# kornelski/cavif-rs

Hardware: AMD Instinct MI355X
Metric: MPix/s encoded at speed=4 q=80, 1080p batch; bit-exact vs CPU oracle (higher is better)
Workload: dtype u16 samples / i32 transform / i64 RD cost

## Files before the change

### __graft_entry__.py

```python
import os
import subprocess
import sys

ROOT = os.path.dirname(os.path.abspath(__file__))
sys.path.insert(0, ROOT)

HIPCC_FLAGS = ['--offload-arch=gfx950', '-O2', '-mllvm', '-sink-insts-to-avoid-spills', '-mllvm', '-inline-threshold=1000', '-mllvm', '-disable-machine-licm', '-mllvm', '-phi-node-folding-threshold=1', '-std=c++17', '-ffp-contract=off', '-fPIC', '-shared', '-Wno-unused-variable']


def _digest(sources, flags):
    import hashlib
    h = hashlib.sha256(' '.join(flags).encode())
    for s in sorted(sources):
        with open(s, 'rb') as fh:
            h.update(os.path.basename(s).encode() + b'\0' + fh.read())
    return h.hexdigest()


def _stale(target, sources):
    if not os.path.exists(target):
        return True
    t = os.path.getmtime(target)
    return any(os.path.getmtime(s) > t for s in sources)

# ... 9 lines not shown
        subprocess.check_call([hipcc] + HIPCC_FLAGS + ['-o', out, os.path.join(csrc, 'mi_avif.hip'), '-lz'])
        with open(stamp, 'w') as fh:
            fh.write(want + '\n')
    cli_src = os.path.join(ROOT, 'cavif_rs_amd', 'cli', 'cavif_mi.cpp')
    cli = os.path.join(ROOT, 'cavif_rs_amd', 'cavif_mi')
    if force or _stale(cli, [cli_src, out, os.path.join(ROOT, 'include', 'mi_avif.h')]):
        subprocess.check_call(['g++', '-O2', '-std=c++17', '-o', cli, cli_src, '-L' + os.path.join(ROOT, 'cavif_rs_amd'), '-lmi_avif', '-lpthread', '-Wl,-rpath,$ORIGIN'])
    subprocess.check_call(['make', '-s', '-C', os.path.join(ROOT, 'oracle')])
    try:
        from tests import emu
        emu.build(force=force)
    except Exception as e:
        print('warning: tests/emu build failed (%s); the -m "not gpu" emulator tests will fail, the product library is unaffected' % e, file=sys.stderr)
    try:
        from tests.helpers import k4_harness
        k4_harness.build_all(force=force)
    except Exception as e:
        print('warning: tests/kernels harness build failed (%s); tests/test_k4_coder.py will fail, the product library is unaffected' % e, file=sys.stderr)
    try:
        from tests.helpers import filters_harness
        filters_harness.build_all(force=force)
    except Exception as e:
        print('warning: tests/kernels filter harness build failed (%s); tests/test_loopfilter_kernels.py will fail, the product library is unaffected' % e, file=sys.stderr)
    try:
        from tests.helpers import predict_harness
        predict_harness.build_all(force=force)
    except Exception as e:
        print('warning: tests/kernels prediction harness build failed (%s); tests/test_predict_kernels.py will fail, the product library is unaffected' % e, file=sys.stderr)
    try:
        from tests.helpers import k1_lookups_harness
        k1_lookups_harness.build_all(force=force)
    except Exception as e:
        print('warning: tests/kernels lookup harness build failed (%s); tests/test_k1_lookups.py will fail, the product library is unaffected' % e, file=sys.stderr)
    import cavif_rs_amd
    cavif_rs_amd.load_library()


def smoke():
    import numpy as np
    import cavif_rs_amd as m
    from cavif_rs_amd.synth import synth_image
    from tests.helpers import oracle
    assert m.device_count() >= 1, 'no HIP device visible'
    img = synth_image(256, 192, index=3)
    enc = m.Encoder().with_quality(80).with_speed(4).with_bit_depth(10)
    got = enc.encode_rgb(img)
    ref, cs, _ = oracle.ravif_encode(img, quality=80, speed=4, depth=10)
    assert got.avif_file[4:12] == b'ftypavif'
    assert got.avif_file == ref, 'HIP path and CPU oracle disagree (%d vs %d bytes)' % (len(got.avif_file), len(ref))
    print('smoke ok: %dx%d -> %d bytes (colour %d), identical to the oracle' % (img.shape[1], img.shape[0], len(got.avif_file), got.color_byte_size))


if __name__ == '__main__':
    build(force='--force' in sys.argv)
    if '--smoke' in sys.argv:
        smoke()
```

### cavif_rs_amd/csrc/dev_common.h

```cpp
#pragma once
#include <hip/hip_runtime.h>
#include <stdint.h>
#include <stddef.h>
#include "av1_tables.h"

#define MI_TX_DEPTH_MAX 2
#define MI_MAX_TILE_COLS 64
#define MI_MAX_TILE_ROWS 64

enum { BS_4 = 0, BS_8 = 1, BS_16 = 2, BS_32 = 3, BS_64 = 4 };
enum { BS_4X8 = 5, BS_8X4 = 6 };
enum { DC_PRED = 0, V_PRED, H_PRED, D45_PRED, D135_PRED, D113_PRED, D157_PRED, D203_PRED, D67_PRED,
       SMOOTH_PRED, SMOOTH_V_PRED, SMOOTH_H_PRED, PAETH_PRED, UV_CFL_PRED };
enum { DCT_DCT = 0, ADST_DCT, DCT_ADST, ADST_ADST, FLIPADST_DCT, DCT_FLIPADST, FLIPADST_FLIPADST,
       ADST_FLIPADST, FLIPADST_ADST, IDTX, V_DCT, H_DCT, V_ADST, H_ADST, V_FLIPADST, H_FLIPADST };
enum { TXC_2D = 0, TXC_HORIZ = 1, TXC_VERT = 2 };

#define MI_SEG_BINS 4096
struct SegTab {
  int n, mean, thr[7], qidx[8], pad_[3];
  struct Q { int dc_q[3], ac_q[3]; uint32_t dc_recip[3], ac_recip[3]; } q[8];
};
struct FrameDev {
  int w, h, bd, np;
// ... 56 lines not shown
__device__ __forceinline__ int imax_(int a, int b) { return a > b ? a : b; }
__device__ __forceinline__ int iclamp_(int v, int lo, int hi) { return v < lo ? lo : (v > hi ? hi : v); }
__device__ __forceinline__ int iabs_(int a) { return a < 0 ? -a : a; }
__device__ __forceinline__ int round2_(int x, int n) { return n == 0 ? x : (x + (1 << (n - 1))) >> n; }
__device__ __forceinline__ int dim_wl(int code) { return code <= 4 ? 2 + code : (code == 5 ? 2 : 3); }
__device__ __forceinline__ int dim_hl(int code) { return code <= 4 ? 2 + code : (code == 5 ? 3 : 2); }

__device__ __forceinline__ int lut4(unsigned long long tab, int i) { return (int)((tab >> (4 * i)) & 15); }
__device__ __forceinline__ int lut8(unsigned long long tab, int i) { return (int)((tab >> (8 * i)) & 255); }
__device__ __forceinline__ int mode_angle_of(int m) { return m == 8 ? 67 : lut8(0xcb9d71872db45a00ULL, m); }
__device__ __forceinline__ int intra_mode_ctx(int m) { return lut4(0x210344443210ULL, m); }

__device__ __forceinline__ int uni32(int v) { return __builtin_amdgcn_readfirstlane(v); }
__device__ __forceinline__ long long uni64(long long v) {
  return (long long)(((unsigned long long)(uint32_t)uni32((int)((unsigned long long)v >> 32)) << 32) | (uint32_t)uni32((int)v));
}

#define DPP_(old, v, ctrl, rmask) __builtin_amdgcn_update_dpp((int)(old), (int)(v), (ctrl), (rmask), 0xF, false)
__device__ __forceinline__ int wave_sum_i32(int v) {
  v += DPP_(0, v, 0xB1, 0xF); v += DPP_(0, v, 0x4E, 0xF); v += DPP_(0, v, 0x141, 0xF); v += DPP_(0, v, 0x140, 0xF);
  v += DPP_(0, v, 0x142, 0xA); v += DPP_(0, v, 0x143, 0xC);
  return __builtin_amdgcn_readlane(v, 63);
}
__device__ __forceinline__ int wave_max_i32(int v) {
  v = imax_(v, DPP_(v, v, 0xB1, 0xF)); v = imax_(v, DPP_(v, v, 0x4E, 0xF)); v = imax_(v, DPP_(v, v, 0x141, 0xF)); v = imax_(v, DPP_(v, v, 0x140, 0xF));
  v = imax_(v, DPP_(v, v, 0x142, 0xA)); v = imax_(v, DPP_(v, v, 0x143, 0xC));
  return __builtin_amdgcn_readlane(v, 63);
}
__device__ __forceinline__ int wave_or_i32(int v) {
  v |= DPP_(0, v, 0xB1, 0xF); v |= DPP_(0, v, 0x4E, 0xF); v |= DPP_(0, v, 0x141, 0xF); v |= DPP_(0, v, 0x140, 0xF);
  v |= DPP_(0, v, 0x142, 0xA); v |= DPP_(0, v, 0x143, 0xC);
  return __builtin_amdgcn_readlane(v, 63);
}
__device__ __forceinline__ long long wave_sum_i64(long long v) {
  const int lo = wave_sum_i32((int)(v & 0xFFFFFF)), hi = wave_sum_i32((int)(v >> 24));
  return ((long long)hi << 24) + (long long)lo;
}
#define WAVE_SYNC() do { __builtin_amdgcn_fence(__ATOMIC_ACQ_REL, "wavefront"); __builtin_amdgcn_wave_barrier(); } while (0)
#define WG_SYNC() __syncthreads()

struct TileB { int mi_row_start, mi_row_end, mi_col_start, mi_col_end; };

__device__ __forceinline__ int seg_ilog2_q11(uint32_t x) {
  if (x == 0) x = 1;
  const int msb = 31 - __clz((int)x);
  unsigned long long m = (unsigned long long)x << (31 - msb);
  int frac = 0;
#pragma unroll
  for (int i = 0; i < 11; i++) { m = (m * m) >> 31; frac <<= 1; if (m >> 32) { frac |= 1; m >>= 1; } }
  return (msb << 11) | frac;
}
__device__ __forceinline__ int seg_bucket(uint32_t scale_q14) { return iclamp_((seg_ilog2_q11(scale_q14) - (6 << 11)) >> 3, 0, MI_SEG_BINS - 1); }
__device__ __forceinline__ int seg_pred(int ul, int u, int l, int *ctx) {
  *ctx = ul < 0 ? 0 : ((ul == u && ul == l) ? 2 : ((ul == u || ul == l || u == l) ? 1 : 0));
  if (u == -1) return l == -1 ? 0 : l;
  if (l == -1) return u;
  return ul == u ? u : l;
}
__device__ __forceinline__ int seg_neg_deinterleave(int diff, int ref, int max) {
  if (!ref) return diff;
  if (ref >= max - 1) return max - diff - 1;
  if (2 * ref < max) { if (diff <= 2 * ref) return (diff & 1) ? ref + ((diff + 1) >> 1) : ref - (diff >> 1); return diff; }
  if (diff <= 2 * (max - ref - 1)) return (diff & 1) ? ref + ((diff + 1) >> 1) : ref - (diff >> 1);
  return max - (diff + 1);
}
__device__ __forceinline__ int seg_symbol(int seg, int pred, int max) {
// ... 91 lines not shown
```

### cavif_rs_amd/csrc/dev_group.h

```cpp
#pragma once
#include "dev_predict.h"
#include "dev_txfm.h"
#include "dev_rate.h"

struct GroupBuf8 {
  int32_t tbuf[8 * 9];
  int32_t cbuf[64];
  int32_t qc[64];
  uint16_t rec[64];
  uint8_t lev[144];
};
#define GROUP_LANE (LANE & 15)
#define GROUP_ID (LANE >> 4)

template <int CTRL> __device__ __forceinline__ int dpp_row_(int v) { return __builtin_amdgcn_update_dpp(0, v, CTRL, 0xF, 0xF, false); }
__device__ __forceinline__ int row_sum_i32(int v) { v += dpp_row_<0x128>(v); v += dpp_row_<0x124>(v); v += dpp_row_<0x122>(v); v += dpp_row_<0x121>(v); return v; }
__device__ __forceinline__ int row_max_i32(int v) {
  v = imax_(v, dpp_row_<0x128>(v)); v = imax_(v, dpp_row_<0x124>(v)); v = imax_(v, dpp_row_<0x122>(v)); v = imax_(v, dpp_row_<0x121>(v)); return v;
}

static __device__ const int tx4_tab[2][3][4][8] = {
  { { { 2896, 2896, 2896, 2896, 0, 0, 0, 0 }, { 3784, 1567, -1567, -3784, 0, 0, 0, 0 }, { 2896, -2896, -2896, 2896, 0, 0, 0, 0 }, { 1567, -3784, 3784, -1567, 0, 0, 0, 0 } },
    { { 1321, 2482, 3344, 3803, 0, 0, 0, 0 }, { 3344, 3344, 0, -3344, 0, 0, 0, 0 }, { 3803, -1321, -3344, 2482, 0, 0, 0, 0 }, { 2482, -3803, 3344, -1321, 0, 0, 0, 0 } },
    { { 5793, 0, 0, 0, 0, 0, 0, 0 }, { 0, 5793, 0, 0, 0, 0, 0, 0 }, { 0, 0, 5793, 0, 0, 0, 0, 0 }, { 0, 0, 0, 5793, 0, 0, 0, 0 } } },
// ... 329 lines not shown
    buf[i - 1] = (uint16_t)((s + 8) >> 4);
  }
  WAVE_SYNC();
}
__device__ __forceinline__ void edge_upsample_group(LDS uint16_t *buf, int num_px, int on, int bd, LDS uint16_t *tmp, int gl) {
  if (on) for (int i = gl; i < num_px + 3; i += 16) {
    uint16_t v;
    if (i == 0) v = buf[-1]; else if (i == num_px + 2) v = buf[num_px - 1]; else v = buf[i - 2];
    tmp[i] = v;
  }
  WAVE_SYNC();
  const int mx = (1 << bd) - 1;
  if (on) {
    if (gl == 0) buf[-2] = tmp[0];
    for (int i = gl; i < num_px; i += 16) {
      int s = -(int)tmp[i] + 9 * (int)tmp[i + 1] + 9 * (int)tmp[i + 2] - (int)tmp[i + 3];
      s = iclamp_(round2_(s, 4), 0, mx);
      buf[2 * i - 1] = (uint16_t)s;
      buf[2 * i] = tmp[i + 2];
    }
  }
  WAVE_SYNC();
}

template <int N>
__device__ inline void predict_dir_group(const LDS FrameDev *f, int x, int y, int have_left, int have_above, int pa, int ftype,
                                         const LDS uint16_t *ra, const LDS uint16_t *rl, LDS GroupPredBuf *gp, LDS uint16_t *out = nullptr) {
  constexpr int log2w = N == 4 ? 2 : 3, nn = N * N;
  const int gl = GROUP_LANE, bd = f->bd;
  const int max_x = f->mi_cols * 4 - 1, max_y = f->mi_rows * 4 - 1;
  LDS uint16_t *wa = gp->wa + EDGE_OFF, *wl = gp->wl + EDGE_OFF;
  for (int i = gl; i < 2 * N + 1; i += 16) { wa[i - 1] = ra[i - 1]; wl[i - 1] = rl[i - 1]; }
  WAVE_SYNC();
  const int diag = pa != 90 && pa != 180;
  {
    const int st_a = (diag && have_above) ? edge_strength_dev(N, N, ftype, pa - 90) : 0;
    const int num_a = imin_(N, max_x - x + 1) + (pa < 90 ? N : 0) + 1;
    edge_filter_group(wa, num_a, st_a, gp->tmp, gl);
    const int st_l = (diag && have_left) ? edge_strength_dev(N, N, ftype, pa - 180) : 0;
    const int num_l = imin_(N, max_y - y + 1) + (pa > 180 ? N : 0) + 1;
    edge_filter_group(wl, num_l, st_l, gp->tmp, gl);
  }
  const int up_a = edge_upsample_sel_dev(N, N, ftype, pa - 90);
  edge_upsample_group(wa, N + (pa < 90 ? N : 0), up_a, bd, gp->tmp, gl);
  const int up_l = edge_upsample_sel_dev(N, N, ftype, pa - 180);
  edge_upsample_group(wl, N + (pa > 180 ? N : 0), up_l, bd, gp->tmp, gl);
  int dx = 0, dy = 0;
#pragma unroll
  for (int r = 0; r < 4; r++) {
    int sdx, sdy;
    dr_dxdy_uni(__builtin_amdgcn_readlane(pa, 16 * r), &sdx, &sdy);
    dx = GROUP_ID == r ? sdx : dx; dy = GROUP_ID == r ? sdy : dy;
  }
  for (int idx = gl; idx < nn; idx += 16) {
    const int i = idx >> log2w, j = idx & (N - 1);
    int v;
    if (pa < 90) {
      const int max_base = (2 * N - 1) << up_a;
      const int id = (i + 1) * dx, base = (id >> (6 - up_a)) + (j << up_a), sh = ((id << up_a) >> 1) & 0x1F;
      v = base < max_base ? round2_(wa[base] * (32 - sh) + wa[base + 1] * sh, 5) : wa[max_base];
    } else if (pa > 90 && pa < 180) {
      int id = (j << 6) - (i + 1) * dx, base = id >> (6 - up_a);
      if (base >= -(1 << up_a)) { const int sh = ((id << up_a) >> 1) & 0x1F; v = round2_(wa[base] * (32 - sh) + wa[base + 1] * sh, 5); }
      else { id = (i << 6) - (j + 1) * dy; base = id >> (6 - up_l); const int sh = ((id << up_l) >> 1) & 0x1F; v = round2_(wl[base] * (32 - sh) + wl[base + 1] * sh, 5); }
    } else if (pa > 180) {
      const int id = (j + 1) * dy, base = (id >> (6 - up_l)) + (i << up_l), sh = ((id << up_l) >> 1) & 0x1F;
      v = round2_(wl[base] * (32 - sh) + wl[base + 1] * sh, 5);
    } else if (pa == 90) v = wa[j];
    else v = wl[i];
    (out ? out : (LDS uint16_t *)gp->pred)[idx] = (uint16_t)v;
  }
  WAVE_SYNC();
}

template <int N>
__device__ inline void predict_nondir_group(int mode, int have_left, int have_above, int bd, const LDS uint16_t *ra, const LDS uint16_t *rl, LDS uint16_t *pred) {
  constexpr int log2w = N == 4 ? 2 : 3, IT = N * N / 16;
  constexpr unsigned long long wt = N == 4 ? 0x405595FFULL : 0x202532496992C5FFULL;
  const int gl = GROUP_LANE;
  if (mode == DC_PRED) {
    int v = 1 << (bd - 1);
    if (have_left || have_above) {
      int s = gl < N ? (have_above ? (int)ra[gl] : 0) + (have_left ? (int)rl[gl] : 0) : 0;
      s = row_sum_i32(s);
      v = (have_left && have_above) ? (s + N) >> (log2w + 1) : (s + (N >> 1)) >> log2w;
    }
// ... 53 lines not shown
```

### cavif_rs_amd/csrc/dev_predict.h

```cpp
#pragma once
#include "dev_common.h"

#define EDGE_OFF 16
#define EDGE_LEN(N) (EDGE_OFF + 2 * (N) + 16)

__device__ __forceinline__ const uint8_t *sm_weights_dev(int log2w) {
  static __device__ const uint8_t sw[124] = { 255, 149, 85, 64,
                                              255, 197, 146, 105, 73, 50, 37, 32,
                                              255, 225, 196, 170, 145, 123, 102, 84, 68, 54, 43, 33, 26, 20, 17, 16,
                                              255, 240, 225, 210, 196, 182, 169, 157, 145, 133, 122, 111, 101, 92, 83, 74,
                                              66, 59, 52, 45, 39, 34, 29, 25, 21, 17, 14, 12, 10, 9, 8, 8,
                                              255, 248, 240, 233, 225, 218, 210, 203, 196, 189, 182, 176, 169, 163, 156, 150,
                                              144, 138, 133, 127, 121, 116, 111, 106, 101, 96, 91, 86, 82, 77, 73, 69,
                                              65, 61, 57, 54, 50, 47, 44, 41, 38, 35, 32, 29, 27, 25, 22, 20,
                                              18, 16, 15, 13, 12, 10, 9, 8, 7, 6, 6, 5, 5, 4, 4, 4 };
  const int l = ((log2w >= 2) & (log2w <= 5)) ? log2w : 6;
  return sw + ((1 << l) - 4);
}
__device__ __forceinline__ int dr_deriv_dev(int a) {
  const int aa = (unsigned)a < 90u ? a : 0;
  const int k = (aa * 43) >> 7;
  const unsigned long long w01 = k < 8 ? 0x97b2d7117423ff00ULL : 0x4047505a00667484ULL, w23 = k < 24 ? 0x171b1f23282d3339ULL : 0x000003070b000f13ULL;
  const unsigned long long w = k < 16 ? w01 : w23;
  const int v = lut8(w, k & 7) | ((int)((0x16cULL >> (2 * k)) & 3) << 8);
  const int r = (int)((0xf035554000eaaa03ULL >> (2 * k)) & 3);
  return aa - 3 * k == r ? v : 0;
}
__device__ __forceinline__ int edge_strength_dev(int w, int h, int ft, int delta) {
  const int d = imin_(iabs_(delta), 254), blk = w + h;
  const int c = (blk > 8) + (blk > 12) + (blk > 16) + (blk > 24) + (blk > 32);
  const unsigned long long t1 = ft == 0 ? 0x010108282838ULL : 0x010104141428ULL, t2 = ft == 0 ? 0x010410ffffffULL : 0x010104303040ULL;
  const unsigned long long t3 = ft == 0 ? 0x012020ffffffULL : 0x010104ffffffULL;
  return (d >= lut8(t1, c)) + (d >= lut8(t2, c)) + (d >= lut8(t3, c));
}
__device__ __forceinline__ int edge_upsample_sel_dev(int w, int h, int ft, int delta) {
  const int d = iabs_(delta), blk = w + h;
  return (int)((d > 0) & (d < 40) & (blk <= (ft == 0 ? 16 : 8)));
}
__device__ __forceinline__ void dr_dxdy_dev(int pa, int *dx, int *dy) {
  *dx = dr_deriv_dev(pa < 90 ? pa : 180 - pa);
  *dy = dr_deriv_dev(pa < 180 ? pa - 90 : 270 - pa);
}
static __device__ const uint32_t dr_dxdy_tab[91] = {
    0x300000, 0x0003ff, 0x000223, 0x000174, 0x200111, 0x2000d7, 0x2000b2, 0x200097, 0x200084, 0x200074, 0x200066, 0x300000, 0x00005a,
    0x000050, 0x000047, 0x000040, 0x000039, 0x000033, 0x00002d, 0x100028, 0x100023, 0x10001f, 0x10001b, 0x100017, 0x100013, 0x10000f,
    0x300000, 0x00000b, 0x000007, 0x000003, 0x300000, 0x0ffc03, 0x088c07, 0x05d00b, 0x24440f, 0x235c13, 0x22c817, 0x225c1b, 0x22101f,
    0x21d023, 0x219828, 0x300000, 0x01682d, 0x014033, 0x011c39, 0x010040, 0x00e447, 0x00cc50, 0x00b45a, 0x10a066, 0x108c74, 0x107c84,
    0x106c97, 0x105cb2, 0x104cd7, 0x103d11, 0x300000, 0x002d74, 0x001e23, 0x000fff, 0x300000, 0x000c00, 0x001c00, 0x002c00, 0x203c00,
    0x204c00, 0x205c00, 0x206c00, 0x207c00, 0x208c00, 0x20a000, 0x300000, 0x00b400, 0x00cc00, 0x00e400, 0x010000, 0x011c00, 0x014000,
    0x016800, 0x119800, 0x11d000, 0x121000, 0x125c00, 0x12c800, 0x135c00, 0x144400, 0x300000, 0x05d000, 0x088c00, 0x0ffc00, 0x300000 };
__device__ __forceinline__ void dr_dxdy_uni(int pa, int *dx, int *dy) {
  const int p = (unsigned)pa <= 270u ? pa : 0, k = (p * 683) >> 11;
  const uint32_t e = dr_dxdy_tab[k];
  const bool has = p - 3 * k == (int)(e >> 20);
  *dx = has ? (int)(e & 1023) : 0; *dy = has ? (int)((e >> 10) & 1023) : 0;
}

__device__ inline void load_edges(const LDS FrameDev *f, int plane, int x, int y, int n, int have_left, int have_above,
                                  int have_ar, int have_bl, LDS uint16_t *above , LDS uint16_t *left) {
  const int bd = f->bd, rs = f->stride;
  const uint16_t *rec = f->rec[plane];
  const int max_x = f->mi_cols * 4 - 1, max_y = f->mi_rows * 4 - 1;
  const int tot = 2 * n;
  const int na = x + (have_ar ? 2 * n : n) - 1, nl = y + (have_bl ? 2 * n : n) - 1;
  const int lim_a = imin_(max_x, na), lim_l = imin_(max_y, nl);
  for (int i = LANE; i <= tot; i += 64) {
    const bool corner = i == tot;
    int ia, il;
    if (have_above) ia = (y - 1) * rs + (corner ? (have_left ? x - 1 : x) : imin_(lim_a, x + i));
    else ia = y * rs + (have_left ? x - 1 : x);
    if (have_left) il = imin_(lim_l, y + i) * rs + x - 1;
    else il = (have_above ? y - 1 : y) * rs + x;
    uint16_t a = rec[ia], l = rec[il];
    if (!have_above && !have_left) { a = (uint16_t)(corner ? (1 << (bd - 1)) : (1 << (bd - 1)) - 1); l = (uint16_t)((1 << (bd - 1)) + 1); }
    if (corner) { above[-1] = a; left[-1] = a; }
    else { above[i] = a; left[i] = l; }
  }
  WAVE_SYNC();
}

__device__ inline void edge_filter_dev(LDS uint16_t *buf, int sz, int strength, LDS uint16_t *tmp) {
  if (!strength) return;
  for (int i = LANE; i < sz; i += 64) tmp[i] = buf[i - 1];
  WAVE_SYNC();
  for (int i = 1 + LANE; i < sz; i += 64) {
    int s = 0;
#pragma unroll
    for (int j = 0; j < 5; j++) {
      const int k = iclamp_(i - 2 + j, 0, sz - 1);
// ... 124 lines not shown
```

### cavif_rs_amd/csrc/dev_rect.h

```cpp
#pragma once

__device__ inline void load_edges_wh(const LDS FrameDev *f, int plane, int x, int y, int w, int h, int have_left, int have_above, int have_ar, int have_bl,
                                     LDS uint16_t *above, LDS uint16_t *left) {
  const int bd = f->bd, rs = f->stride, tot = w + h;
  const uint16_t *rec = f->rec[plane];
  const int max_x = f->mi_cols * 4 - 1, max_y = f->mi_rows * 4 - 1;
  const int lim_a = imin_(max_x, x + (have_ar ? 2 * w : w) - 1), lim_l = imin_(max_y, y + (have_bl ? 2 * h : h) - 1);
  for (int i = LANE; i <= tot; i += 64) {
    const bool corner = i == tot;
    int ia, il;
    if (have_above) ia = (y - 1) * rs + (corner ? (have_left ? x - 1 : x) : imin_(lim_a, x + i));
    else ia = y * rs + (have_left ? x - 1 : x);
    if (have_left) il = imin_(lim_l, y + i) * rs + x - 1;
    else il = (have_above ? y - 1 : y) * rs + x;
    uint16_t a = rec[ia], l = rec[il];
    if (!have_above && !have_left) { a = (uint16_t)(corner ? (1 << (bd - 1)) : (1 << (bd - 1)) - 1); l = (uint16_t)((1 << (bd - 1)) + 1); }
    if (corner) { above[-1] = a; left[-1] = a; } else { above[i] = a; left[i] = l; }
  }
  WAVE_SYNC();
}

__device__ inline void predict_block_wh(const LDS FrameDev *f, int x, int y, int wl, int hl, int have_left, int have_above, int mode, int angle_delta, int ftype,
                                        const LDS uint16_t *ra, const LDS uint16_t *rl, LDS uint16_t *wa, LDS uint16_t *wl_, LDS uint16_t *tmp, LDS uint16_t *pred) {
  const int w = 1 << wl, h = 1 << hl, bd = f->bd, nn = w * h;
// ... 718 lines not shown
        }
        if (W == 0 && LANE < 2) {
          const int rr = r + (H_ == 8 ? LANE : 0), cc = c + (W_ == 8 ? LANE : 0), o = rr * ms + cc;
          f->m_txsize[o] = 0; f->m_txtype[o] = (uint8_t)sub[LANE * 4 + 0]; f->m_eob[0][o] = (uint16_t)sub[LANE * 4 + 1];
          f->m_lvl[0][o] = (uint8_t)sub[LANE * 4 + 2]; f->m_dc[0][o] = (uint8_t)sub[LANE * 4 + 3];
        }
      } else if (W == 0 && LANE < 2) {
        const int o = (r + (H_ == 8 ? LANE : 0)) * ms + c + (W_ == 8 ? LANE : 0);
        f->m_lvl[0][o] = (uint8_t)SH->lm_tx; f->m_dc[0][o] = (uint8_t)SH->lm_delta;
      }
      WG_SYNC();
    }
  }
  if (luma_j >= budget) return luma_j;
  long long total_j = luma_j;
  PH(13);
  bool cgrouped = false;
  if constexpr (CAN_GROUP) cgrouped = f->np > 1 && !Tools<TS>::FULL;
  if constexpr (CAN_GROUP) if (cgrouped) {
    const uint16_t *uvcost = k.cost() + CDF_UV_CFL + best_mode * CDF_UV_CFL_STRIDE;
    const int nplain = best_mode != DC_PRED ? 2 : 1, nc = nplain + 1, uvset = Tools<TS>::reduced_tx_set(f) ? 2 : 1;
    const int mx = (1 << f->bd) - 1;
    {
      const int p = (W >> 1) + 1, half = W & 1;
      const LDS uint16_t *luma = SH->luma_rec;
      int lsum = LANE < NN ? (int)luma[LANE] << 3 : 0;
      lsum = wave_sum_i32(lsum);
      const int avg = round2_(lsum, WL + HL);
      predict_block_wh(f, x, y, WL, HL, availL, availU, DC_PRED, 0, ftype_uv, SH->ra[p] + EDGE_OFF, SH->rl[p] + EDGE_OFF, wa, wl, S->etmp, S->dcp);
      long long best_sse = J_INF; int best_idx = 1 << 20;
      const int l = LANE < NN ? ((int)luma[LANE] << 3) - avg : 0, dcv = LANE < NN ? (int)S->dcp[LANE] : 0, sv = LANE < NN ? (int)SH->srcb[p][LANE] : 0;
      if (half == 0) { const int d = sv - dcv; best_sse = (long long)wave_sum_i32(LANE < NN ? d * d : 0); best_idx = -1; }
      const int la = iabs_(l), ng = l < 0;
#pragma unroll
      for (int kq = 0; kq < 8; kq++) {
        const int mag = half * 8 + kq + 1;
        const int rr = round2_(__mul24(mag, la), 6), sc = ng ? -rr : rr;
        const int dp = sv - iclamp_(dcv + sc, 0, mx), dm = sv - iclamp_(dcv - sc, 0, mx);
        const long long ep = (long long)wave_sum_i32(LANE < NN ? __mul24(dp, dp) : 0), em = (long long)wave_sum_i32(LANE < NN ? __mul24(dm, dm) : 0);
        if (ep < best_sse) { best_sse = ep; best_idx = half * 16 + 2 * kq; }
        if (em < best_sse) { best_sse = em; best_idx = half * 16 + 2 * kq + 1; }
      }
      if (LANE == 0) { SH->ca_sse[p - 1][half] = best_sse; SH->ca_idx[p - 1][half] = best_idx; }
    }
    WG_SYNC();
    int alpha_u = 0, alpha_v = 0;
#pragma unroll
    for (int pp = 0; pp < 2; pp++) {
      const int idx = SH->ca_sse[pp][1] < SH->ca_sse[pp][0] ? SH->ca_idx[pp][1] : SH->ca_idx[pp][0];
      const int al = idx < 0 ? 0 : ((idx & 1) ? -((idx >> 1) + 1) : ((idx >> 1) + 1));
      if (pp == 0) alpha_u = al; else alpha_v = al;
    }
    const int cfl_ok = alpha_u != 0 || alpha_v != 0;
    GroupRes gr = { 0, 0, 0, 0, 0 };
    const int cw = (W & 1) == 0;
    if (!cw && nplain == 2) {
      const int p = (W >> 1) + 1;
      predict_block_wh(f, x, y, WL, HL, availL, availU, best_mode, 0, ftype_uv, SH->ra[p] + EDGE_OFF, SH->rl[p] + EDGE_OFF, wa, wl, S->etmp, k.wave(W - 1)->pred + NN);
    }
    if (cw) {
      const int p = (W >> 1) + 1;
      {
        const int al = p == 1 ? alpha_u : alpha_v;
        LDS uint16_t *cp = S->pred + (nc - 1) * NN;
        int lsum = LANE < NN ? (int)SH->luma_rec[LANE] << 3 : 0;
        lsum = wave_sum_i32(lsum);
        const int avg = round2_(lsum, WL + HL);
        if (LANE < NN) { const int l = ((int)SH->luma_rec[LANE] << 3) - avg, v = al * l, sc = v >= 0 ? round2_(v, 6) : -round2_(-v, 6); cp[LANE] = (uint16_t)iclamp_((int)S->dcp[LANE] + sc, 0, mx); }
      }
      WAVE_SYNC();
    }
    WG_SYNC();
    if (cw) {
      const int p = (W >> 1) + 1;
      const int g = GROUP_ID, cand = imin_(g, nc - 1);
// ... 29 lines not shown
        fill_rect<WL, HL>((uint8_t *)f->m_angle_uv, ms, r, c, 0);
        fill_rect<WL, HL>(f->m_cfl_sign, ms, r, c, chose_cfl ? b_sign : 0);
        fill_rect<WL, HL>(f->m_cfl_au, ms, r, c, (chose_cfl && alpha_u) ? iabs_(alpha_u) - 1 : 0);
        fill_rect<WL, HL>(f->m_cfl_av, ms, r, c, (chose_cfl && alpha_v) ? iabs_(alpha_v) - 1 : 0);
      }
    }
    WG_SYNC();
    any_coef |= (SH->ceob[0] > 0) | (SH->ceob[1] > 0);
    total_j += best_uv;
  }
  if constexpr (Tools<TS>::FULL) if (f->np > 1 && !cgrouped) {
    const uint16_t *uvcost = k.cost() + CDF_UV_CFL + best_mode * CDF_UV_CFL_STRIDE;
    unsigned long long cand_pack = 0; int nc = 0;
    auto push = [&](int m) { cand_pack |= (unsigned long long)m << (4 * nc); nc++; };
    push(DC_PRED);
    if (best_mode != DC_PRED) push(best_mode);
    if (Tools<TS>::FULL) for (int m = 1; m < 13; m++) if (m != best_mode) push(m);
    push(UV_CFL_PRED);
    const int uvset = Tools<TS>::reduced_tx_set(f) ? 2 : 1;
    const int mx = (1 << f->bd) - 1;
    const int p = (W >> 1) + 1, half = W & 1;
    const LDS uint16_t *pra = SH->ra[p] + EDGE_OFF, *prl = SH->rl[p] + EDGE_OFF;
    int lavg;
    {
      const LDS uint16_t *luma = SH->luma_rec;
      int lsum = LANE < NN ? (int)luma[LANE] << 3 : 0;
      lsum = wave_sum_i32(lsum);
      lavg = round2_(lsum, WL + HL);
      predict_block_wh(f, x, y, WL, HL, availL, availU, DC_PRED, 0, ftype_uv, pra, prl, wa, wl, S->etmp, S->dcp);
      long long best_sse = J_INF; int best_idx = 1 << 20;
      const int l = LANE < NN ? ((int)luma[LANE] << 3) - lavg : 0, dcv = LANE < NN ? (int)S->dcp[LANE] : 0, sv = LANE < NN ? (int)SH->srcb[p][LANE] : 0;
      if (half == 0) { const int d = sv - dcv; best_sse = (long long)wave_sum_i32(LANE < NN ? d * d : 0); best_idx = -1; }
      const int la = iabs_(l), ng = l < 0;
#pragma unroll
      for (int kq = 0; kq < 8; kq++) {
        const int mag = half * 8 + kq + 1;
        const int rr = round2_(__mul24(mag, la), 6), sc = ng ? -rr : rr;
        const int dp = sv - iclamp_(dcv + sc, 0, mx), dm = sv - iclamp_(dcv - sc, 0, mx);
        const long long ep = (long long)wave_sum_i32(LANE < NN ? __mul24(dp, dp) : 0), em = (long long)wave_sum_i32(LANE < NN ? __mul24(dm, dm) : 0);
        if (ep < best_sse) { best_sse = ep; best_idx = half * 16 + 2 * kq; }
        if (em < best_sse) { best_sse = em; best_idx = half * 16 + 2 * kq + 1; }
      }
      if (LANE == 0) { SH->ca_sse[p - 1][half] = best_sse; SH->ca_idx[p - 1][half] = best_idx; }
    }
    WG_SYNC();
    int alpha_u = 0, alpha_v = 0;
#pragma unroll
    for (int pp = 0; pp < 2; pp++) {
      const int idx = SH->ca_sse[pp][1] < SH->ca_sse[pp][0] ? SH->ca_idx[pp][1] : SH->ca_idx[pp][0];
      const int al = idx < 0 ? 0 : ((idx & 1) ? -((idx >> 1) + 1) : ((idx >> 1) + 1));
      if (pp == 0) alpha_u = al; else alpha_v = al;
    }
    const int cfl_ok = alpha_u != 0 || alpha_v != 0;
    LDS uint16_t *park_rec = (LDS uint16_t *)SH->lpred + (p - 1) * 96; LDS int32_t *park_qc = (LDS int32_t *)(park_rec + 32); LDS int *park_meta = (LDS int *)SH->order + (p - 1) * 3;
    long long best_uv = J_INF; int b_ci = 1 << 30, b_sign = 0, b_round = 0;
    const int ns = nc <= 4 ? 1 : 2, nrounds = nc > 4 * ns ? 2 : 1, dealt = half < ns;
    GroupRes gr = { 0, 0, 0, 0, 0 };
    const int g = GROUP_ID;
#pragma unroll 1
    for (int rd = 0; rd < nrounds; rd++) {
      const int base = nrounds == 2 && rd == 0 ? 4 * ns : 0;
#pragma unroll 1
      for (int g2 = 0; g2 < 4; g2++) {
        const int ci = base + half + ns * g2;
        if (dealt && ci < nc) {
          const int um = lut4(cand_pack, ci);
          LDS uint16_t *cp = S->pred + g2 * NN;
          if (um == UV_CFL_PRED) {
            const int al = p == 1 ? alpha_u : alpha_v;
            if (LANE < NN) { const int l = ((int)SH->luma_rec[LANE] << 3) - lavg, v = al * l, sc = v >= 0 ? round2_(v, 6) : -round2_(-v, 6); cp[LANE] = (uint16_t)iclamp_((int)S->dcp[LANE] + sc, 0, mx); }
            WAVE_SYNC();
          } else if (um != DC_PRED) predict_block_wh(f, x, y, WL, HL, availL, availU, um, 0, ftype_uv, pra, prl, wa, wl, S->etmp, cp);
        }
      }
      const int ci = base + half + ns * g, live = dealt && ci < nc;
// ... 65 lines not shown
```

### cavif_rs_amd/csrc/tile_search.h

```cpp
#pragma once
#include "dev_common.h"
#include "dev_predict.h"
#include "dev_txfm.h"
#include "dev_rate.h"
#include "dev_group.h"

#ifndef MI_BALLOT64
#define MI_BALLOT64(p) __builtin_amdgcn_ballot_w64(p)
#endif
#define MI_K1_TRY_ATTR __attribute__((noinline, not_tail_called))
#define MI_K1_WG_PER_CU 4
#define WAVE_ID ((int)(threadIdx.x >> 6))
#ifndef MI_PROFILE
#define MI_PROFILE 0
#endif
#ifndef MI_PROF_MAXN
#define MI_PROF_MAXN 16
#endif
#ifndef MI_DEBUG_HOOKS
#define MI_DEBUG_HOOKS 0
#endif
#if MI_DEBUG_HOOKS
#define DBG_IS(f, v) ((f)->dbg == (v))
#else
// ... 885 lines not shown
  if constexpr (SMALL_GROUPED) if (cgrouped) {
    const uint16_t *uvcost = k.cost() + CDF_UV_CFL + best_mode * CDF_UV_CFL_STRIDE;
    const int nplain = best_mode != DC_PRED ? 2 : 1, nc = nplain + 1, uvset = tx_set_of(BS, Tools<TS>::reduced_tx_set(f));
    const int bdelta = (best_mode >= V_PRED && best_mode <= D67_PRED && BS >= BS_8) ? best_delta : 0;
    const int mx = (1 << f->bd) - 1;
    {
      const int p = (W >> 1) + 1, half = W & 1;
      const LDS uint16_t *luma = SH->luma_rec;
      int lsum = 0;
      for (int idx = LANE; idx < nn; idx += 64) lsum += luma[idx] << 3;
      lsum = wave_sum_i32(lsum);
      const int avg = round2_(lsum, 2 * log2w);
      predict_block(f, x, y, log2w, availL, availU, DC_PRED, 0, ftype_uv, SH->ra[p] + EDGE_OFF, SH->rl[p] + EDGE_OFF, wa, wl, S->etmp, S->dcp);
      long long best_sse = J_INF; int best_idx = 1 << 20;
      if (half == 0) {
        int e0 = 0;
        for (int idx = LANE; idx < nn; idx += 64) { const int d = (int)SH->srcb[p][idx] - (int)S->dcp[idx]; e0 += __mul24(d, d); }
        best_sse = (long long)wave_sum_i32(e0); best_idx = -1;
      }
      int e[16];
#pragma unroll
      for (int a = 0; a < 16; a++) e[a] = 0;
      for (int idx = LANE; idx < nn; idx += 64) {
        const int l = ((int)luma[idx] << 3) - avg, dcv = S->dcp[idx], sv = SH->srcb[p][idx];
        const int la = iabs_(l), neg = l < 0;
#pragma unroll
        for (int kq = 0; kq < 8; kq++) {
          const int mag = half * 8 + kq + 1;
          const int rr = round2_(__mul24(mag, la), 6), sc = neg ? -rr : rr;
          const int dp = sv - iclamp_(dcv + sc, 0, mx), dm = sv - iclamp_(dcv - sc, 0, mx);
          e[2 * kq] += __mul24(dp, dp); e[2 * kq + 1] += __mul24(dm, dm);
        }
      }
#pragma unroll
      for (int a = 0; a < 16; a++) {
        const long long ea = (long long)wave_sum_i32(e[a]);
        if (ea < best_sse) { best_sse = ea; best_idx = half * 16 + a; }
      }
      if (LANE == 0) { SH->ca_sse[p - 1][half] = best_sse; SH->ca_idx[p - 1][half] = best_idx; }
    }
    PH(8);
    WG_SYNC();
    PH(2);
    int alpha_u = 0, alpha_v = 0;
#pragma unroll
    for (int pp = 0; pp < 2; pp++) {
      const int idx = SH->ca_sse[pp][1] < SH->ca_sse[pp][0] ? SH->ca_idx[pp][1] : SH->ca_idx[pp][0];
      const int al = idx < 0 ? 0 : ((idx & 1) ? -((idx >> 1) + 1) : ((idx >> 1) + 1));
      if (pp == 0) alpha_u = al; else alpha_v = al;
    }
    const int cfl_ok = alpha_u != 0 || alpha_v != 0;
    GroupRes gr = { 0, 0, 0, 0, 0 };
    const int cw = (W & 1) == 0;
    if (!cw && nplain == 2) {
      const int p = (W >> 1) + 1;
      predict_block(f, x, y, log2w, availL, availU, best_mode, bdelta, ftype_uv, SH->ra[p] + EDGE_OFF, SH->rl[p] + EDGE_OFF, wa, wl, S->etmp, k.wave(W - 1)->pred + nn);
    }
    if (cw) {
      const int p = (W >> 1) + 1;
      {
        const int al = p == 1 ? alpha_u : alpha_v;
        LDS uint16_t *cp = S->pred + (nc - 1) * nn;
        int lsum = 0;
        for (int idx = LANE; idx < nn; idx += 64) lsum += SH->luma_rec[idx] << 3;
        lsum = wave_sum_i32(lsum);
        const int avg = round2_(lsum, 2 * log2w);
        for (int idx = LANE; idx < nn; idx += 64) {
          const int l = ((int)SH->luma_rec[idx] << 3) - avg, v = al * l, sc = v >= 0 ? round2_(v, 6) : -round2_(-v, 6);
          cp[idx] = (uint16_t)iclamp_((int)S->dcp[idx] + sc, 0, mx);
        }
      }
// ... 63 lines not shown
    push(UV_CFL_PRED);
    const int uvset = tx_set_of(BS, Tools<TS>::reduced_tx_set(f));
    const int mx = (1 << f->bd) - 1;
    const int p = (W >> 1) + 1, half = W & 1;
    const LDS uint16_t *pra = SH->ra[p] + EDGE_OFF, *prl = SH->rl[p] + EDGE_OFF;
    int lavg;
    {
      const LDS uint16_t *luma = SH->luma_rec;
      int lsum = 0;
      for (int idx = LANE; idx < nn; idx += 64) lsum += luma[idx] << 3;
      lsum = wave_sum_i32(lsum);
      lavg = round2_(lsum, 2 * log2w);
      predict_block(f, x, y, log2w, availL, availU, DC_PRED, 0, ftype_uv, pra, prl, wa, wl, S->etmp, S->dcp);
      long long best_sse = J_INF; int best_idx = 1 << 20;
      if (half == 0) {
        int e0 = 0;
        for (int idx = LANE; idx < nn; idx += 64) { const int d = (int)SH->srcb[p][idx] - (int)S->dcp[idx]; e0 += __mul24(d, d); }
        best_sse = (long long)wave_sum_i32(e0); best_idx = -1;
      }
      int e[16];
#pragma unroll
      for (int a2 = 0; a2 < 16; a2++) e[a2] = 0;
      for (int idx = LANE; idx < nn; idx += 64) {
        const int l = ((int)luma[idx] << 3) - lavg, dcv = S->dcp[idx], sv = SH->srcb[p][idx];
        const int la = iabs_(l), neg = l < 0;
#pragma unroll
        for (int kq = 0; kq < 8; kq++) {
          const int mag = half * 8 + kq + 1;
          const int rr = round2_(__mul24(mag, la), 6), sc = neg ? -rr : rr;
          const int dp = sv - iclamp_(dcv + sc, 0, mx), dm = sv - iclamp_(dcv - sc, 0, mx);
          e[2 * kq] += __mul24(dp, dp); e[2 * kq + 1] += __mul24(dm, dm);
        }
      }
#pragma unroll
      for (int a2 = 0; a2 < 16; a2++) {
        const long long ea = (long long)wave_sum_i32(e[a2]);
        if (ea < best_sse) { best_sse = ea; best_idx = half * 16 + a2; }
      }
      if (LANE == 0) { SH->ca_sse[p - 1][half] = best_sse; SH->ca_idx[p - 1][half] = best_idx; }
    }
    PH(8);
    WG_SYNC();
    PH(2);
    int alpha_u = 0, alpha_v = 0;
#pragma unroll
    for (int pp = 0; pp < 2; pp++) {
      const int idx = SH->ca_sse[pp][1] < SH->ca_sse[pp][0] ? SH->ca_idx[pp][1] : SH->ca_idx[pp][0];
      const int al = idx < 0 ? 0 : ((idx & 1) ? -((idx >> 1) + 1) : ((idx >> 1) + 1));
      if (pp == 0) alpha_u = al; else alpha_v = al;
    }
    const int cfl_ok = alpha_u != 0 || alpha_v != 0;
    LDS uint16_t *park_rec = (LDS uint16_t *)SH->lpred + (p - 1) * 3 * nn; LDS int32_t *park_qc = (LDS int32_t *)(park_rec + nn); LDS int *park_meta = (LDS int *)SH->order + (p - 1) * 3;
    static_assert(2 * 3 * nn <= 768, "the parked candidates fit lpred");
    long long best_uv = J_INF; int b_ci = 1 << 30, b_sign = 0, b_round = 0, b_delta = 0;
    const int ns = nc <= 4 ? 1 : 2, nrounds = nc > 4 * ns ? 2 : 1, dealt = half < ns;
    GroupRes gr = { 0, 0, 0, 0, 0 };
    const int g = GROUP_ID;
    auto delta_of = [&](int um) { return (um == best_mode && um >= V_PRED && um <= D67_PRED && BS >= BS_8) ? best_delta : 0; };
#pragma unroll 1
    for (int rd = 0; rd < nrounds; rd++) {
      const int base = nrounds == 2 && rd == 0 ? 4 * ns : 0;
#pragma unroll 1
      for (int g2 = 0; g2 < 4; g2++) {
        const int ci = base + half + ns * g2;
        if (dealt && ci < nc) {
          const int um = lut4(cand_pack, ci);
          LDS uint16_t *cp = S->pred + g2 * nn;
          if (um == UV_CFL_PRED) {
            const int al = p == 1 ? alpha_u : alpha_v;
            for (int idx = LANE; idx < nn; idx += 64) {
              const int l = ((int)SH->luma_rec[idx] << 3) - lavg, v = al * l, sc = v >= 0 ? round2_(v, 6) : -round2_(-v, 6);
// ... 88 lines not shown
      if (txtype_to_sym(uvset, txtype) < 0) txtype = DCT_DCT;
      {
        const int p = (W & 1) + 1;
        const int cfl_main = valid && um == UV_CFL_PRED;
        const int cfl_help = cfl_allowed && active && pair == 0 && rd == nother - 1;
        if (cfl_main || cfl_help) {
          const int half = cfl_help ? 1 : 0;
          const LDS uint16_t *luma = SH->luma_rec;
          int lsum = 0;
          for (int idx = LANE; idx < nn; idx += 64) lsum += luma[idx] << 3;
          lsum = wave_sum_i32(lsum);
          const int avg = round2_(lsum, 2 * log2w), mx = (1 << f->bd) - 1;
          predict_block(f, x, y, log2w, availL, availU, DC_PRED, 0, ftype_uv, SH->ra[p] + EDGE_OFF, SH->rl[p] + EDGE_OFF, wa, wl, S->etmp, S->dcp);
          long long best_sse = J_INF; int best_idx = 1 << 20;
          if (half == 0) {
            int e0 = 0;
            for (int idx = LANE; idx < nn; idx += 64) { const int d = (int)SH->srcb[p][idx] - (int)S->dcp[idx]; e0 += __mul24(d, d); }
            best_sse = wave_sum_i64((long long)e0); best_idx = -1;
          }
          int e[16];
#pragma unroll
          for (int a = 0; a < 16; a++) e[a] = 0;
          for (int idx = LANE; idx < nn; idx += 64) {
            const int l = ((int)luma[idx] << 3) - avg, dcv = S->dcp[idx], sv = SH->srcb[p][idx];
            const int la = iabs_(l), neg = l < 0;
#pragma unroll
            for (int kq = 0; kq < 8; kq++) {
              const int mag = half * 8 + kq + 1;
              const int r = round2_(__mul24(mag, la), 6), sc = neg ? -r : r;
              const int dp = sv - iclamp_(dcv + sc, 0, mx), dm = sv - iclamp_(dcv - sc, 0, mx);
              e[2 * kq] += __mul24(dp, dp); e[2 * kq + 1] += __mul24(dm, dm);
            }
          }
#pragma unroll
          for (int a = 0; a < 16; a++) {
            const long long ea = (long long)wave_sum_i32(e[a]);
            if (ea < best_sse) { best_sse = ea; best_idx = half * 16 + a; }
          }
          if (LANE == 0) { SH->ca_sse[p - 1][half] = best_sse; SH->ca_idx[p - 1][half] = best_idx; }
        }
      }
      PH(8);
      WG_SYNC();
      PH(2);
      int alpha_u = 0, alpha_v = 0, jsign = 0, ok = valid;
      if (valid && um == UV_CFL_PRED) {
#pragma unroll
        for (int pp = 0; pp < 2; pp++) {
          const int idx = SH->ca_sse[pp][1] < SH->ca_sse[pp][0] ? SH->ca_idx[pp][1] : SH->ca_idx[pp][0];
          const int al = idx < 0 ? 0 : ((idx & 1) ? -((idx >> 1) + 1) : ((idx >> 1) + 1));
          if (pp == 0) alpha_u = al; else alpha_v = al;
        }
        if (alpha_u == 0 && alpha_v == 0) ok = 0;
      }
      const uint32_t mode_rate = uv_mode_rate(k.cost(), uvcost, um, um >= V_PRED && um <= D67_PRED && BS >= BS_8, delta,
                                              valid && um == UV_CFL_PRED && ok, alpha_u, alpha_v, &jsign);
      TxRes trp = { 0, 0, 0, 0, 0 };
      if (ok) {
        {
          const int p = (W & 1) + 1;
          const LDS uint16_t *pra = SH->ra[p] + EDGE_OFF, *prl = SH->rl[p] + EDGE_OFF;
          if (um == UV_CFL_PRED) {
            const int al = p == 1 ? alpha_u : alpha_v;
            predict_block(f, x, y, log2w, availL, availU, DC_PRED, 0, ftype_uv, pra, prl, wa, wl, S->etmp, S->dcp);
            if (al) {
              int lsum = 0;
              for (int idx = LANE; idx < nn; idx += 64) lsum += SH->luma_rec[idx] << 3;
              lsum = wave_sum_i32(lsum);
              const int avg = round2_(lsum, 2 * log2w), mx = (1 << f->bd) - 1;
              for (int idx = LANE; idx < nn; idx += 64) {
                const int l = ((int)SH->luma_rec[idx] << 3) - avg, v = al * l, sc = v >= 0 ? round2_(v, 6) : -round2_(-v, 6);
// ... 447 lines not shown
```

Measured before the change: 558.2.

## Fold sixteen CfL SSE reductions into one butterfly argmin and tabulate DR edge params

```diff
diff --git a/__graft_entry__.py b/__graft_entry__.py
--- a/__graft_entry__.py
+++ b/__graft_entry__.py
@@ -65,6 +65,11 @@
         k1_lookups_harness.build_all(force=force)
     except Exception as e:
         print('warning: tests/kernels lookup harness build failed (%s); tests/test_k1_lookups.py will fail, the product library is unaffected' % e, file=sys.stderr)
+    try:
+        from tests.helpers import k1_serial_harness
+        k1_serial_harness.build_all(force=force)
+    except Exception as e:
+        print('warning: tests/kernels serial-path harness build failed (%s); tests/test_k1_serial_path.py will fail, the product library is unaffected' % e, file=sys.stderr)
     import cavif_rs_amd
     cavif_rs_amd.load_library()
 
diff --git a/cavif_rs_amd/csrc/dev_common.h b/cavif_rs_amd/csrc/dev_common.h
--- a/cavif_rs_amd/csrc/dev_common.h
+++ b/cavif_rs_amd/csrc/dev_common.h
@@ -112,6 +112,54 @@
   v |= DPP_(0, v, 0x142, 0xA); v |= DPP_(0, v, 0x143, 0xC);
   return __builtin_amdgcn_readlane(v, 63);
 }
+__device__ __forceinline__ int wave_min_i32(int v) {
+  v = imin_(v, DPP_(v, v, 0xB1, 0xF)); v = imin_(v, DPP_(v, v, 0x4E, 0xF)); v = imin_(v, DPP_(v, v, 0x141, 0xF)); v = imin_(v, DPP_(v, v, 0x140, 0xF));
+  v = imin_(v, DPP_(v, v, 0x142, 0xA)); v = imin_(v, DPP_(v, v, 0x143, 0xC));
+  return __builtin_amdgcn_readlane(v, 63);
+}
+template <int BIT> __device__ __forceinline__ int fold_pair(int a, int b) {
+  static_assert(BIT >= 2 && BIT <= 5, "fold_pair: lane bits 2..5");
+  if constexpr (BIT >= 4) {
+#ifdef MI_EMU
+    const int hi = (LANE >> BIT) & 1, keep = hi ? b : a, give = hi ? a : b;
+    return keep + __shfl(give, LANE ^ (1 << BIT));
+#else
+    typedef unsigned fold_v2u_ __attribute__((ext_vector_type(2)));
+    fold_v2u_ s;
+    if constexpr (BIT == 5) s = __builtin_amdgcn_permlane32_swap((unsigned)a, (unsigned)b, false, false);
+    else s = __builtin_amdgcn_permlane16_swap((unsigned)a, (unsigned)b, false, false);
+    return (int)(s.x + s.y);
+#endif
+  } else {
+    constexpr int N = 1 << BIT, LO = BIT == 3 ? 0x3 : 0x5, HI = BIT == 3 ? 0xC : 0xA;
+    const int t = __builtin_amdgcn_update_dpp(b, a, 0x100 + N, 0xF, LO, false);
+    const int u = __builtin_amdgcn_update_dpp(a, b, 0x110 + N, 0xF, HI, false);
+    return t + u;
+  }
+}
+__device__ __forceinline__ int fold16_slot() { return ((LANE >> 2) & 1) << 3 | ((LANE >> 3) & 1) << 2 | ((LANE >> 4) & 1) << 1 | ((LANE >> 5) & 1); }
+__device__ __forceinline__ int wave_fold16_i32(const int (&e)[16]) {
+  int f8[8], f4[4], f2[2];
+#pragma unroll
+  for (int j = 0; j < 8; j++) f8[j] = fold_pair<5>(e[2 * j], e[2 * j + 1]);
+#pragma unroll
+  for (int j = 0; j < 4; j++) f4[j] = fold_pair<4>(f8[2 * j], f8[2 * j + 1]);
+#pragma unroll
+  for (int j = 0; j < 2; j++) f2[j] = fold_pair<3>(f4[2 * j], f4[2 * j + 1]);
+  int v = fold_pair<2>(f2[0], f2[1]);
+  v += DPP_(0, v, 0xB1, 0xF); v += DPP_(0, v, 0x4E, 0xF);
+  return v;
+}
+__device__ __forceinline__ void wave_argmin16_i32(const int (&e)[16], int *best, int *idx) {
+  const int v = wave_fold16_i32(e), m = wave_min_i32(v);
+  *best = m;
+  *idx = wave_min_i32(v == m ? fold16_slot() : 16);
+}
+__device__ __forceinline__ void cfl_scan_tail(const int (&e)[16], int half, long long *best_sse, int *best_idx) {
+  int fm, fa;
+  wave_argmin16_i32(e, &fm, &fa);
+  if ((long long)fm < *best_sse) { *best_sse = fm; *best_idx = half * 16 + fa; }
+}
 __device__ __forceinline__ long long wave_sum_i64(long long v) {
   const int lo = wave_sum_i32((int)(v & 0xFFFFFF)), hi = wave_sum_i32((int)(v >> 24));
   return ((long long)hi << 24) + (long long)lo;
diff --git a/cavif_rs_amd/csrc/dev_group.h b/cavif_rs_amd/csrc/dev_group.h
--- a/cavif_rs_amd/csrc/dev_group.h
+++ b/cavif_rs_amd/csrc/dev_group.h
@@ -385,26 +385,28 @@
   LDS uint16_t *wa = gp->wa + EDGE_OFF, *wl = gp->wl + EDGE_OFF;
   for (int i = gl; i < 2 * N + 1; i += 16) { wa[i - 1] = ra[i - 1]; wl[i - 1] = rl[i - 1]; }
   WAVE_SYNC();
-  const int diag = pa != 90 && pa != 180;
+  uint32_t rp = 0;
   {
-    const int st_a = (diag && have_above) ? edge_strength_dev(N, N, ftype, pa - 90) : 0;
+    const int sft = uni32(ftype);
+#pragma unroll
+    for (int r = 0; r < 4; r++) {
+      const uint32_t srp = dr_row_uni(__builtin_amdgcn_readlane(pa, 16 * r), log2w, sft);
+      rp = GROUP_ID == r ? srp : rp;
+    }
+  }
+  const int dx = dr_row_dx(rp), dy = dr_row_dy(rp);
+  {
+    const int st_a = have_above ? dr_row_strength_above(rp) : 0;
     const int num_a = imin_(N, max_x - x + 1) + (pa < 90 ? N : 0) + 1;
     edge_filter_group(wa, num_a, st_a, gp->tmp, gl);
-    const int st_l = (diag && have_left) ? edge_strength_dev(N, N, ftype, pa - 180) : 0;
+    const int st_l = have_left ? dr_row_strength_left(rp) : 0;
     const int num_l = imin_(N, max_y - y + 1) + (pa > 180 ? N : 0) + 1;
     edge_filter_group(wl, num_l, st_l, gp->tmp, gl);
   }
-  const int up_a = edge_upsample_sel_dev(N, N, ftype, pa - 90);
+  const int up_a = dr_row_upsample_above(rp);
   edge_upsample_group(wa, N + (pa < 90 ? N : 0), up_a, bd, gp->tmp, gl);
-  const int up_l = edge_upsample_sel_dev(N, N, ftype, pa - 180);
+  const int up_l = dr_row_upsample_left(rp);
   edge_upsample_group(wl, N + (pa > 180 ? N : 0), up_l, bd, gp->tmp, gl);
-  int dx = 0, dy = 0;
-#pragma unroll
-  for (int r = 0; r < 4; r++) {
-    int sdx, sdy;
-    dr_dxdy_uni(__builtin_amdgcn_readlane(pa, 16 * r), &sdx, &sdy);
-    dx = GROUP_ID == r ? sdx : dx; dy = GROUP_ID == r ? sdy : dy;
-  }
   for (int idx = gl; idx < nn; idx += 16) {
     const int i = idx >> log2w, j = idx & (N - 1);
     int v;
diff --git a/cavif_rs_amd/csrc/dev_predict.h b/cavif_rs_amd/csrc/dev_predict.h
--- a/cavif_rs_amd/csrc/dev_predict.h
+++ b/cavif_rs_amd/csrc/dev_predict.h
@@ -41,20 +41,42 @@
   *dx = dr_deriv_dev(pa < 90 ? pa : 180 - pa);
   *dy = dr_deriv_dev(pa < 180 ? pa - 90 : 270 - pa);
 }
-static __device__ const uint32_t dr_dxdy_tab[91] = {
-    0x300000, 0x0003ff, 0x000223, 0x000174, 0x200111, 0x2000d7, 0x2000b2, 0x200097, 0x200084, 0x200074, 0x200066, 0x300000, 0x00005a,
-    0x000050, 0x000047, 0x000040, 0x000039, 0x000033, 0x00002d, 0x100028, 0x100023, 0x10001f, 0x10001b, 0x100017, 0x100013, 0x10000f,
-    0x300000, 0x00000b, 0x000007, 0x000003, 0x300000, 0x0ffc03, 0x088c07, 0x05d00b, 0x24440f, 0x235c13, 0x22c817, 0x225c1b, 0x22101f,
-    0x21d023, 0x219828, 0x300000, 0x01682d, 0x014033, 0x011c39, 0x010040, 0x00e447, 0x00cc50, 0x00b45a, 0x10a066, 0x108c74, 0x107c84,
-    0x106c97, 0x105cb2, 0x104cd7, 0x103d11, 0x300000, 0x002d74, 0x001e23, 0x000fff, 0x300000, 0x000c00, 0x001c00, 0x002c00, 0x203c00,
-    0x204c00, 0x205c00, 0x206c00, 0x207c00, 0x208c00, 0x20a000, 0x300000, 0x00b400, 0x00cc00, 0x00e400, 0x010000, 0x011c00, 0x014000,
-    0x016800, 0x119800, 0x11d000, 0x121000, 0x125c00, 0x12c800, 0x135c00, 0x144400, 0x300000, 0x05d000, 0x088c00, 0x0ffc00, 0x300000 };
+static __device__ const uint32_t dr_dxdy_tab[91][2] = {
+    { 0x300000, 0x00000000 }, { 0x0003ff, 0xff285285 }, { 0x000223, 0xff285285 }, { 0x000174, 0xff285285 }, { 0x200111, 0xff285285 }, { 0x2000d7, 0xff285285 },
+    { 0x2000b2, 0xff285285 }, { 0x200097, 0xff285285 }, { 0x200084, 0xff285285 }, { 0x200074, 0xff285245 }, { 0x200066, 0xff285245 }, { 0x300000, 0x00000000 },
+    { 0x00005a, 0xff285244 }, { 0x000050, 0xff285244 }, { 0x000047, 0xff285244 }, { 0x000040, 0xff245244 }, { 0x000039, 0xff245244 }, { 0x000033, 0xff254614 },
+    { 0x00002d, 0xff254614 }, { 0x100028, 0xff254614 }, { 0x100023, 0xfe254614 }, { 0x10001f, 0xfe254614 }, { 0x10001b, 0xfe254614 }, { 0x100017, 0xfe254614 },
+    { 0x100013, 0xfe214614 }, { 0x10000f, 0xfe214614 }, { 0x300000, 0x00000000 }, { 0x00000b, 0xfe214614 }, { 0x000007, 0xfe214614 }, { 0x000003, 0xfd214614 },
+    { 0x300000, 0x00000000 }, { 0x0ffc03, 0xfd214614 }, { 0x088c07, 0xfe214614 }, { 0x05d00b, 0xfe214614 }, { 0x24440f, 0xfe214614 }, { 0x235c13, 0xfe214614 },
+    { 0x22c817, 0xfe254614 }, { 0x225c1b, 0xfe254614 }, { 0x22101f, 0xfe254614 }, { 0x21d023, 0xfe254514 }, { 0x219828, 0xff254514 }, { 0x300000, 0x00000000 },
+    { 0x01682d, 0xff254510 }, { 0x014033, 0xff254510 }, { 0x011c39, 0xff245140 }, { 0x010040, 0xff145140 }, { 0x00e447, 0xff185140 }, { 0x00cc50, 0xff1a1860 },
+    { 0x00b45a, 0xff1a1860 }, { 0x10a066, 0xff1a1861 }, { 0x108c74, 0xfb1a1861 }, { 0x107c84, 0xfb1a18a1 }, { 0x106c97, 0xfb1a18a1 }, { 0x105cb2, 0xfb1a18a1 },
+    { 0x104cd7, 0xfb0a18a1 }, { 0x103d11, 0xfb0a18a1 }, { 0x300000, 0x00000000 }, { 0x002d74, 0xfb0a18a1 }, { 0x001e23, 0xfb0a18a1 }, { 0x000fff, 0xf70a18a1 },
+    { 0x300000, 0x00000000 }, { 0x000c00, 0xf70a18a1 }, { 0x001c00, 0xfb0a18a1 }, { 0x002c00, 0xfb0a18a1 }, { 0x203c00, 0xfb0a18a1 }, { 0x204c00, 0xfb0a18a1 },
+    { 0x205c00, 0xfb1a18a1 }, { 0x206c00, 0xfb1a18a1 }, { 0x207c00, 0xfb1a18a1 }, { 0x208c00, 0xfb1a18a1 }, { 0x20a000, 0xff1a18a1 }, { 0x300000, 0x00000000 },
+    { 0x00b400, 0xff1a18a1 }, { 0x00cc00, 0xff1a18a1 }, { 0x00e400, 0xff185181 }, { 0x010000, 0xff185181 }, { 0x011c00, 0xff285181 }, { 0x014000, 0xff285181 },
+    { 0x016800, 0xff285181 }, { 0x119800, 0xff285185 }, { 0x11d000, 0xff285185 }, { 0x121000, 0xff285285 }, { 0x125c00, 0xff285285 }, { 0x12c800, 0xff285285 },
+    { 0x135c00, 0xff285285 }, { 0x144400, 0xff285285 }, { 0x300000, 0x00000000 }, { 0x05d000, 0xff285285 }, { 0x088c00, 0xff285285 }, { 0x0ffc00, 0xff285285 },
+    { 0x300000, 0x00000000 } };
 __device__ __forceinline__ void dr_dxdy_uni(int pa, int *dx, int *dy) {
   const int p = (unsigned)pa <= 270u ? pa : 0, k = (p * 683) >> 11;
-  const uint32_t e = dr_dxdy_tab[k];
+  const uint32_t e = dr_dxdy_tab[k][0];
   const bool has = p - 3 * k == (int)(e >> 20);
   *dx = has ? (int)(e & 1023) : 0; *dy = has ? (int)((e >> 10) & 1023) : 0;
 }
+__device__ __forceinline__ uint32_t dr_row_uni(int pa, int log2n, int ft) {
+  const int p = (unsigned)pa <= 270u ? pa : 0, k = (p * 683) >> 11;
+  const uint32_t e = dr_dxdy_tab[k][0], g = dr_dxdy_tab[k][1];
+  const bool has = p - 3 * k == (int)(e >> 20);
+  const uint32_t fld = log2n == 4 ? (g >> (24 + 4 * ft)) & 15 : (g >> (6 * (2 * (log2n - 2) + ft))) & 63;
+  return has ? (e & 0xFFFFF) | fld << 20 : 0;
+}
+__device__ __forceinline__ int dr_row_dx(uint32_t rp) { return (int)(rp & 1023); }
+__device__ __forceinline__ int dr_row_dy(uint32_t rp) { return (int)((rp >> 10) & 1023); }
+__device__ __forceinline__ int dr_row_strength_above(uint32_t rp) { return (int)((rp >> 20) & 3); }
+__device__ __forceinline__ int dr_row_strength_left(uint32_t rp) { return (int)((rp >> 22) & 3); }
+__device__ __forceinline__ int dr_row_upsample_above(uint32_t rp) { return (int)((rp >> 24) & 1); }
+__device__ __forceinline__ int dr_row_upsample_left(uint32_t rp) { return (int)((rp >> 25) & 1); }
 
 __device__ inline void load_edges(const LDS FrameDev *f, int plane, int x, int y, int n, int have_left, int have_above,
                                   int have_ar, int have_bl, LDS uint16_t *above , LDS uint16_t *left) {
diff --git a/cavif_rs_amd/csrc/dev_rect.h b/cavif_rs_amd/csrc/dev_rect.h
--- a/cavif_rs_amd/csrc/dev_rect.h
+++ b/cavif_rs_amd/csrc/dev_rect.h
@@ -774,15 +774,15 @@
       const int l = LANE < NN ? ((int)luma[LANE] << 3) - avg : 0, dcv = LANE < NN ? (int)S->dcp[LANE] : 0, sv = LANE < NN ? (int)SH->srcb[p][LANE] : 0;
       if (half == 0) { const int d = sv - dcv; best_sse = (long long)wave_sum_i32(LANE < NN ? d * d : 0); best_idx = -1; }
       const int la = iabs_(l), ng = l < 0;
+      int e[16];
 #pragma unroll
       for (int kq = 0; kq < 8; kq++) {
         const int mag = half * 8 + kq + 1;
         const int rr = round2_(__mul24(mag, la), 6), sc = ng ? -rr : rr;
         const int dp = sv - iclamp_(dcv + sc, 0, mx), dm = sv - iclamp_(dcv - sc, 0, mx);
-        const long long ep = (long long)wave_sum_i32(LANE < NN ? __mul24(dp, dp) : 0), em = (long long)wave_sum_i32(LANE < NN ? __mul24(dm, dm) : 0);
-        if (ep < best_sse) { best_sse = ep; best_idx = half * 16 + 2 * kq; }
-        if (em < best_sse) { best_sse = em; best_idx = half * 16 + 2 * kq + 1; }
-      }
+        e[2 * kq] = LANE < NN ? __mul24(dp, dp) : 0; e[2 * kq + 1] = LANE < NN ? __mul24(dm, dm) : 0;
+      }
+      cfl_scan_tail(e, half, &best_sse, &best_idx);
       if (LANE == 0) { SH->ca_sse[p - 1][half] = best_sse; SH->ca_idx[p - 1][half] = best_idx; }
     }
     WG_SYNC();
@@ -878,15 +878,15 @@
       const int l = LANE < NN ? ((int)luma[LANE] << 3) - lavg : 0, dcv = LANE < NN ? (int)S->dcp[LANE] : 0, sv = LANE < NN ? (int)SH->srcb[p][LANE] : 0;
       if (half == 0) { const int d = sv - dcv; best_sse = (long long)wave_sum_i32(LANE < NN ? d * d : 0); best_idx = -1; }
       const int la = iabs_(l), ng = l < 0;
+      int e[16];
 #pragma unroll
       for (int kq = 0; kq < 8; kq++) {
         const int mag = half * 8 + kq + 1;
         const int rr = round2_(__mul24(mag, la), 6), sc = ng ? -rr : rr;
         const int dp = sv - iclamp_(dcv + sc, 0, mx), dm = sv - iclamp_(dcv - sc, 0, mx);
-        const long long ep = (long long)wave_sum_i32(LANE < NN ? __mul24(dp, dp) : 0), em = (long long)wave_sum_i32(LANE < NN ? __mul24(dm, dm) : 0);
-        if (ep < best_sse) { best_sse = ep; best_idx = half * 16 + 2 * kq; }
-        if (em < best_sse) { best_sse = em; best_idx = half * 16 + 2 * kq + 1; }
-      }
+        e[2 * kq] = LANE < NN ? __mul24(dp, dp) : 0; e[2 * kq + 1] = LANE < NN ? __mul24(dm, dm) : 0;
+      }
+      cfl_scan_tail(e, half, &best_sse, &best_idx);
       if (LANE == 0) { SH->ca_sse[p - 1][half] = best_sse; SH->ca_idx[p - 1][half] = best_idx; }
     }
     WG_SYNC();
diff --git a/cavif_rs_amd/csrc/tile_search.h b/cavif_rs_amd/csrc/tile_search.h
--- a/cavif_rs_amd/csrc/tile_search.h
+++ b/cavif_rs_amd/csrc/tile_search.h
@@ -941,11 +941,7 @@
           e[2 * kq] += __mul24(dp, dp); e[2 * kq + 1] += __mul24(dm, dm);
         }
       }
-#pragma unroll
-      for (int a = 0; a < 16; a++) {
-        const long long ea = (long long)wave_sum_i32(e[a]);
-        if (ea < best_sse) { best_sse = ea; best_idx = half * 16 + a; }
-      }
+      cfl_scan_tail(e, half, &best_sse, &best_idx);
       if (LANE == 0) { SH->ca_sse[p - 1][half] = best_sse; SH->ca_idx[p - 1][half] = best_idx; }
     }
     PH(8);
@@ -1075,11 +1071,7 @@
           e[2 * kq] += __mul24(dp, dp); e[2 * kq + 1] += __mul24(dm, dm);
         }
       }
-#pragma unroll
-      for (int a2 = 0; a2 < 16; a2++) {
-        const long long ea = (long long)wave_sum_i32(e[a2]);
-        if (ea < best_sse) { best_sse = ea; best_idx = half * 16 + a2; }
-      }
+      cfl_scan_tail(e, half, &best_sse, &best_idx);
       if (LANE == 0) { SH->ca_sse[p - 1][half] = best_sse; SH->ca_idx[p - 1][half] = best_idx; }
     }
     PH(8);
@@ -1234,11 +1226,7 @@
               e[2 * kq] += __mul24(dp, dp); e[2 * kq + 1] += __mul24(dm, dm);
             }
           }
-#pragma unroll
-          for (int a = 0; a < 16; a++) {
-            const long long ea = (long long)wave_sum_i32(e[a]);
-            if (ea < best_sse) { best_sse = ea; best_idx = half * 16 + a; }
-          }
+          cfl_scan_tail(e, half, &best_sse, &best_idx);
           if (LANE == 0) { SH->ca_sse[p - 1][half] = best_sse; SH->ca_idx[p - 1][half] = best_idx; }
         }
       }
```

Result: faster. 564.3 (median of 6 runs) (+1.1%).
